# Quantum-Chemistry-Group-BNU/PyNQS

Measured on AMD Instinct MI355X. Metric: local energies/sec (whole node), higher is better.
Workload: dtype f64

## Files before the change

include/pynqs_amd.h:

```cpp
#ifndef PYNQS_AMD_H
#define PYNQS_AMD_H

#include <stdint.h>

#ifdef __cplusplus
extern "C" {
#endif

#define PYNQS_ABI_VERSION 1

#define PYNQS_OK 0
#define PYNQS_EINVAL (-1)
#define PYNQS_ELAUNCH (-2)
#define PYNQS_ELENGTH (-3)
#define PYNQS_EOVERFLOW (-4)

#define PYNQS_F32 0
#define PYNQS_F64 1

#define PYNQS_MAX_SORB_LEN 3
#define PYNQS_MAX_SORB 192
#define PYNQS_MAX_NELE 120
#define PYNQS_MAX_NVIR 120

// ... 186 lines not shown
} pynqs_reduce_io;
int pynqs_reduce_onepass_geometry(int64_t nbatch, int sorb, int nele, int noA, int noB, int eps_sample, int64_t *out4);
int64_t pynqs_reduce_onepass_tile_scratch_bytes(int64_t nbatch, int sorb, int nele, int noA, int noB, int eps_sample);
int pynqs_reduce_onepass_list_capacity(int64_t nbatch, int sorb, int nele, int noA, int noB, int dtype, int eps_sample,
                                       int with_row_cache, int without_table, int64_t *cap_doubles);
int pynqs_reduce_onepass_wants_row_f32(int64_t nbatch, int sorb, int nele, int noA, int noB, int dtype, int eps_sample, int64_t cap_doubles,
                                       int with_tile_scratch ,
                                       int without_table );
int64_t pynqs_reduce_onepass_row_f32_elements(int64_t nbatch, int sorb, int nele, int noA, int noB);
int pynqs_reduce_onepass(const uint64_t *bra, int64_t nbatch, int sorb, int nele, int noA, int noB, const void *plan,
                         int dtype, double eps, int eps_sample, uint64_t seed, const pynqs_reduce_io *io, void *stream);
int pynqs_reduce_contract(int64_t nbatch, int sorb, int nele, int noA, int noB, int dtype, int eps_sample,
                          const pynqs_reduce_io *io, const double *psi_unique, const double *psi_table, int psi_is_complex,
                          int divide, double *eloc, double *psi_x, void *stream);
#define PYNQS_CONTRACT_BATCHED 0
#define PYNQS_CONTRACT_SERIAL 1
int pynqs_reduce_contract_form(int64_t nbatch, int sorb, int nele, int noA, int noB, int dtype, int eps_sample,
                               const pynqs_reduce_io *io, const double *psi_unique, const double *psi_table, int psi_is_complex,
                               int divide, double *eloc, double *psi_x, int form, void *stream);

#define PYNQS_RBM_COMPLEX 4
int pynqs_rbm_forward(const uint64_t *onv, int64_t n, int sorb, const double *weights, const double *hidden_bias,
                      const double *visible_bias, int nhidden, int flavour, double *psi, void *stream);

int64_t pynqs_rbm_children_table_bytes(int64_t nwalkers, int sorb, int nhidden, int flavour);
int pynqs_rbm_children_prepare(const uint64_t *walkers, int64_t nwalkers, int sorb, const double *weights, const double *hidden_bias,
                               const double *visible_bias, int nhidden, int flavour, void *table, void *stream);
int pynqs_rbm_forward_children(const uint64_t *onv, int64_t n, const int32_t *count_dev, const int32_t *parent,
                               const uint64_t *walkers, int64_t nwalkers, const void *table, int sorb, const double *weights,
                               const double *hidden_bias, const double *visible_bias, int nhidden, int flavour, double *psi,
                               void *stream);
int pynqs_rbm_forward_children_supported(int sorb, int nhidden, int flavour);
int pynqs_rbm_forward_children_geometry(int64_t n, int sorb, int nhidden, int flavour, int64_t *out4);
int pynqs_rbm_children_prepare_stamped(const uint64_t *walkers, int64_t nwalkers, int sorb, const double *weights,
                                       const double *hidden_bias, const double *visible_bias, int nhidden, int flavour, uint64_t stamp,
                                       void *table, void *stream);
int pynqs_rbm_forward_children_stamped(const uint64_t *onv, int64_t n, const int32_t *count_dev, const int32_t *parent,
                                       const uint64_t *walkers, int64_t nwalkers, const void *table, int sorb, const double *weights,
                                       const double *hidden_bias, const double *visible_bias, int nhidden, int flavour, uint64_t stamp,
                                       double *psi, void *stream);

int64_t pynqs_rbm_grad_workspace(int64_t n, int sorb, int nhidden, int flavour);
int pynqs_rbm_grad(const uint64_t *onv, int64_t n, int sorb, const double *weights, const double *hidden_bias,
                   const double *visible_bias, int nhidden, int flavour, const double *prob, const double *eloc,
                   int eloc_is_complex, const double *e_total, const double *pow, double *grad_weights,
                   double *grad_hidden_bias, double *grad_visible_bias, double *loss, void *workspace, void *stream);
int pynqs_rbm_grad_loss(const uint64_t *onv, int64_t n, int sorb, const double *weights, const double *hidden_bias,
                        const double *visible_bias, int nhidden, int flavour, const double *prob, const double *eloc,
                        int eloc_is_complex, const double *e_total, const double *pow, double *grad_weights,
                        double *grad_hidden_bias, double *grad_visible_bias, double *loss, double *loss_copy, void *workspace,
                        void *stream);
#define PYNQS_GRAD_ONEPASS 0
#define PYNQS_GRAD_TWOPASS 1
int pynqs_rbm_grad_loss_form(const uint64_t *onv, int64_t n, int sorb, const double *weights, const double *hidden_bias,
                             const double *visible_bias, int nhidden, int flavour, const double *prob, const double *eloc,
                             int eloc_is_complex, const double *e_total, const double *pow, double *grad_weights,
                             double *grad_hidden_bias, double *grad_visible_bias, double *loss, double *loss_copy, void *workspace,
                             int schedule, int block, void *stream);

#define PYNQS_SR_RHO 0
#define PYNQS_SR_RHS2 1
#define PYNQS_SR_DONE 2
#define PYNQS_SR_ITER 3
#define PYNQS_SR_TRUE2 4
#define PYNQS_SR_PAP 5
#define PYNQS_SR_CONVERGED 6
#define PYNQS_SR_BREAKDOWN 7
#define PYNQS_SR_NSCALARS 8
#define PYNQS_SR_CG_INIT 0
#define PYNQS_SR_CG_STEP 1
#define PYNQS_SR_CG_RESIDUAL 2
int64_t pynqs_rbm_sr_workspace(int64_t n, int sorb, int nhidden, int flavour);
int pynqs_rbm_sr_prepare(const uint64_t *onv, int64_t n, int sorb, const double *weights, const double *hidden_bias, int nhidden,
// ... 41 lines not shown
```

pynqs_amd/C_extension.py:

```python
from __future__ import annotations

import itertools
import os
import warnings
import weakref
from typing import Tuple

import numpy as np
import torch
from torch import Tensor

from . import _native as N

MAX_SORB_LEN = 3
MAX_SORB = 64 * MAX_SORB_LEN
MAX_NELE = 120
USE_PLAN = True

__all__ = [
    "tensor_to_onv", "onv_to_tensor", "get_comb_tensor", "get_hij_torch", "get_comb_hij_fused",
    "wavefunction_lut", "hash_build", "hash_lookup", "HashTable", "RBMTable", "eloc_rbm", "JastrowTable", "eloc_jrbm", "green_jrbm", "jrbm_forward", "eloc_jrbm_supported", "merge_rank_sample", "spin_flip_rand", "check_sorb", "compress_h1e_h2e", "decompress_h1e_h2e", "get_Num_SinglesDoubles",
    "MAX_SORB", "MAX_SORB_LEN", "MAX_NELE",
]

# ... 644 lines not shown
    n = onv.size(0)
    psi = torch.empty(n, dtype=_rbm_dtype(rbm_type), device=onv.device)
    N.check(N.lib().pynqs_rbm_forward(onv.data_ptr(), n, sorb, W.data_ptr(), hb.data_ptr(), vb.data_ptr() if vb is not None else None, H, flav,
                                      psi.data_ptr(), _stream(onv.device)), "pynqs_rbm_forward")
    return psi


def _rbm_params(weights, hidden_bias, visible_bias, sorb, rbm_type, on_gpu=True):
    flav = RBM_TYPE_FLAVOUR.get(rbm_type)
    if flav is None:
        raise RuntimeError(f"rbm_type {rbm_type!r} has no fused forward")
    cplx_par = rbm_type == "complex"
    W = weights.detach().double().contiguous()
    hb = hidden_bias.detach().double().contiguous()
    vb = visible_bias.detach().double().contiguous() if visible_bias is not None else None
    H = W.size(0)
    if W.shape[:2] != (H, sorb) or W.dim() != (3 if cplx_par else 2) or hb.numel() != H * (2 if cplx_par else 1) or \
            (vb is not None and vb.numel() != sorb * (2 if cplx_par else 1)):
        raise RuntimeError("RBM parameter shapes do not match sorb / num_hidden")
    if on_gpu and not (W.is_cuda and hb.is_cuda and (vb is None or vb.is_cuda)):
        raise RuntimeError("RBM parameters must be on the GPU")
    return flav, W, hb, vb, H


def rbm_forward_children_supported(sorb: int, num_hidden: int, rbm_type: str = "real") -> bool:
    flav = RBM_TYPE_FLAVOUR.get(rbm_type)
    return flav is not None and bool(N.lib().pynqs_rbm_forward_children_supported(sorb, num_hidden, flav))


_CHILDREN_STAMP = itertools.count(1)


def rbm_forward_children(onv: Tensor, parent: Tensor, walkers: Tensor, weights: Tensor, hidden_bias: Tensor, visible_bias: "Tensor | None",
                         sorb: int, rbm_type: str = "real", count: "Tensor | None" = None, out: "Tensor | None" = None) -> Tensor:
    _check_onv(onv, "onv", sorb, (2,))
    _check_onv(walkers, "walkers", sorb, (2,))
    flav, W, hb, vb, H = _rbm_params(weights, hidden_bias, visible_bias, sorb, rbm_type)
    dev = onv.device
    if not (onv.is_cuda and walkers.device == dev and parent.device == dev and parent.dtype == torch.int32 and parent.numel() >= onv.size(0)):
        raise RuntimeError("rbm_forward_children: onv, walkers and parent (int32) on one GPU")
    n, nw = onv.size(0), walkers.size(0)
    nbytes = N.lib().pynqs_rbm_children_table_bytes(nw, sorb, H, flav)
    table = torch.empty(max(nbytes // 8, 1), dtype=torch.float64, device=dev)
    st = _stream(dev)
    wk = walkers.contiguous()
    stamp = next(_CHILDREN_STAMP)
    N.check(N.lib().pynqs_rbm_children_prepare_stamped(wk.data_ptr(), nw, sorb, W.data_ptr(), hb.data_ptr(), vb.data_ptr() if vb is not None else None,
                                                       H, flav, stamp, table.data_ptr(), st), "pynqs_rbm_children_prepare_stamped")
    psi = out if out is not None else torch.empty(n, dtype=_rbm_dtype(rbm_type), device=dev)
    N.check(N.lib().pynqs_rbm_forward_children_stamped(onv.contiguous().data_ptr(), n, count.data_ptr() if count is not None else None,
                                                       parent.data_ptr(), wk.data_ptr(), nw, table.data_ptr(), sorb, W.data_ptr(), hb.data_ptr(),
                                                       vb.data_ptr() if vb is not None else None, H, flav, stamp, psi.data_ptr(), st),
            "pynqs_rbm_forward_children_stamped")
    return psi


class CRBMTable(_RBMTableBase):

    def __init__(self, weights: Tensor, hidden_bias: Tensor, visible_bias: "Tensor | None" = None) -> None:
        def as_pairs(t: Tensor) -> Tensor:
            t = t.detach()
            if t.is_complex():
                t = torch.view_as_real(t.to(torch.complex128))
            if t.dtype != torch.float64 or t.size(-1) != 2:
                raise RuntimeError("complex RBM parameters must be complex128 or float64 (re, im) pairs")
            return t.contiguous()

        w, hb = as_pairs(weights), as_pairs(hidden_bias).reshape(-1, 2)
        vb = as_pairs(visible_bias).reshape(-1, 2) if visible_bias is not None else None
        if w.dim() != 3 or hb.size(0) != w.size(0) or (vb is not None and vb.size(0) != w.size(1)):
            raise RuntimeError("weights must be [num_hidden, sorb], hidden_bias [num_hidden], visible_bias [sorb]")
        given = [weights, hidden_bias] + ([visible_bias] if visible_bias is not None else [])
        self._build("crbm", given, [w, hb] + ([vb] if vb is not None else []), int(w.size(0)), int(w.size(1)))


def eloc_crbm(bra: Tensor, h1e: Tensor, h2e: Tensor, table: CRBMTable, sorb: int, nele: int, noA: int, noB: int,
              want_psi: bool = True, log_scale: float = 0.0) -> Tuple[Tensor, "Tensor | None"]:
    _check_onv(bra, "bra", sorb, (2,))
    return _eloc_fused(bra, h1e, h2e, table, sorb, want_psi, torch.complex128, lambda x, n, plan, eloc, psi, st: N.check(
        N.lib().pynqs_eloc_crbm(x.data_ptr(), n, sorb, nele, noA, noB, plan.data_ptr(), table.data_ptr(), table.nhidden, float(log_scale),
                                eloc.data_ptr(), psi, st), "pynqs_eloc_crbm"))


_CHARTS = None


# ... 97 lines not shown
```

pynqs_amd/_native.py:

```python
from __future__ import annotations

import ctypes as C
import os

_HERE = os.path.dirname(os.path.abspath(__file__))
LIB_PATH = os.environ.get("PYNQS_AMD_LIB") or os.path.join(_HERE, "csrc", "libpynqs_amd.so")

PYNQS_F32, PYNQS_F64 = 0, 1
RBM_REAL, RBM_TANH, RBM_PHASE, RBM_COMPLEX = 0, 1, 2, 4
OK, EINVAL, ELAUNCH, ELENGTH, EOVERFLOW = 0, -1, -2, -3, -4

_i64, _int, _vp, _dbl = C.c_int64, C.c_int, C.c_void_p, C.c_double

SIGNATURES = {
    "pynqs_abi_version": (_int, []),
    "pynqs_last_error": (C.c_char_p, []),
    "pynqs_num_sd": (_i64, [_int, _int, _int]),
    "pynqs_check_sorb": (_int, [_int, _int]),
    "pynqs_comb_hij_fused": (_int, [_vp, _i64, _int, _int, _int, _int, _vp, _vp, _int, _vp, _vp, _vp]),
    "pynqs_comb": (_int, [_vp, _i64, _int, _int, _int, _vp, _vp, _vp]),
    "pynqs_hij": (_int, [_vp, _i64, _vp, _i64, _int, _vp, _vp, _int, _int, _int, _vp, _vp]),
    "pynqs_onv_to_pm1": (_int, [_vp, _i64, _int, _int, _vp, _vp]),
    "pynqs_pm01_to_onv": (_int, [_vp, _i64, _int, _vp, _vp]),
    "pynqs_wavefunction_lut": (_int, [_vp, _i64, _vp, _i64, _int, _vp, _vp, _vp]),
    "pynqs_spin_flip_rand": (_int, [_vp, _i64, _int, _int, _int, C.c_uint64, C.c_uint64, _vp, _vp]),
    "pynqs_plan_bytes": (_i64, [_int, _int]),
    "pynqs_plan_build": (_int, [_vp, _vp, _int, _int, _vp, _vp]),
    "pynqs_comb_hij_fused_plan": (_int, [_vp, _i64, _int, _int, _int, _int, _vp, _int, _vp, _vp, _vp]),
    "pynqs_eloc_sample_space": (_int, [_vp, _i64, _int, _int, _int, _int, _vp, _vp, _i64, _vp, _int, _vp, _vp, _vp]),
    "pynqs_hash_bytes": (_i64, [_i64, _int]),
    "pynqs_hash_build": (_int, [_vp, _i64, _int, _vp, _vp]),
    "pynqs_hash_lookup": (_int, [_vp, _i64, _vp, _i64, _int, _vp, _vp, _vp]),
    "pynqs_unique_workspace": (_i64, [_i64]),
    "pynqs_unique_first": (_int, [_vp, _i64, _int, _vp, _vp, _vp]),
    "pynqs_eloc_sample_space_hash": (_int, [_vp, _i64, _int, _int, _int, _int, _vp, _vp, _i64, _vp, _int, _vp, _vp, _vp]),
    "pynqs_eloc_sample_space_flip": (_int, [_vp, _i64, _int, _int, _int, _int, _vp, _vp, _i64, _vp, _int, _vp, _vp, _vp]),
    "pynqs_eloc_sample_space_hash_flip": (_int, [_vp, _i64, _int, _int, _int, _int, _vp, _vp, _i64, _vp, _int, _vp, _vp, _vp]),
    "pynqs_eloc_sample_space_keys": (_int, [_vp, _i64, _int, _int, _int, _int, _vp, _vp, _i64, _vp, _int, _int, _vp, _vp, _vp]),
    "pynqs_keys_index_bytes": (_i64, [_i64, _int]),
    "pynqs_keys_index_workspace": (_i64, [_i64, _int]),
    "pynqs_keys_index_build": (_int, [_vp, _i64, _int, _vp, _vp, _vp]),
    "pynqs_keys_index_density": (_int, [_vp, _i64, _int, _vp, _vp]),
# ... 27 lines not shown
    "pynqs_reduce_tiles": (_i64, [_i64, _int, _int, _int, _int]),
    "pynqs_reduce_count": (_int, [_vp, _i64, _int, _int, _int, _int, _vp, _int, _dbl, _vp, _vp]),
    "pynqs_reduce_count_sums": (_int, [_vp, _i64, _int, _int, _int, _int, _vp, _int, _dbl, _vp, _vp, _vp]),
    "pynqs_reduce_sample": (_int, [_vp, _i64, _int, _int, _int, _int, _vp, _int, _dbl, _vp, _vp, _vp, C.c_uint64, _vp, _vp, _vp, _vp]),
    "pynqs_reduce_emit": (_int, [_vp, _i64, _int, _int, _int, _int, _vp, _int, _dbl, _vp, _vp, _vp, _vp, _vp]),
}



class ReduceIO(C.Structure):
    _fields_ = [("cap_doubles", _i64), ("cap_unique", _i64), ("dedup_slots", _i64),
                ("rec_col", _vp), ("rec_w", _vp), ("rec_onv", _vp), ("rec_link", _vp), ("seg_count", _vp),
                ("srec_col", _vp), ("srec_w", _vp), ("srec_onv", _vp), ("srec_link", _vp), ("row_sum", _vp),
                ("dedup_table", _vp), ("uniq_onv", _vp), ("uniq_pm1", _vp), ("pm1_dtype", C.c_int32), ("lut_is_hash", C.c_int32),
                ("lut_table", _vp), ("lut_nkeys", _i64), ("counters", _vp), ("seed_dev", _vp), ("row_cache", _vp), ("uniq_parent", _vp),
                ("tile_scratch", _vp), ("tile_scratch_bytes", _i64), ("row_f32", _vp)]


SIGNATURES.update({
    "pynqs_reduce_onepass_geometry": (_int, [_i64, _int, _int, _int, _int, _int, C.POINTER(_i64)]),
    "pynqs_reduce_onepass_tile_scratch_bytes": (_i64, [_i64, _int, _int, _int, _int, _int]),
    "pynqs_reduce_onepass_list_capacity": (_int, [_i64, _int, _int, _int, _int, _int, _int, _int, _int, C.POINTER(_i64)]),
    "pynqs_reduce_onepass_wants_row_f32": (_int, [_i64, _int, _int, _int, _int, _int, _int, _i64, _int, _int]),
    "pynqs_reduce_onepass_row_f32_elements": (_i64, [_i64, _int, _int, _int, _int]),
    "pynqs_reduce_onepass": (_int, [_vp, _i64, _int, _int, _int, _int, _vp, _int, _dbl, _int, C.c_uint64, C.POINTER(ReduceIO), _vp]),
    "pynqs_rbm_forward": (_int, [_vp, _i64, _int, _vp, _vp, _vp, _int, _int, _vp, _vp]),
    "pynqs_rbm_children_table_bytes": (_i64, [_i64, _int, _int, _int]),
    "pynqs_rbm_children_prepare": (_int, [_vp, _i64, _int, _vp, _vp, _vp, _int, _int, _vp, _vp]),
    "pynqs_rbm_forward_children": (_int, [_vp, _i64, _vp, _vp, _vp, _i64, _vp, _int, _vp, _vp, _vp, _int, _int, _vp, _vp]),
    "pynqs_rbm_forward_children_supported": (_int, [_int, _int, _int]),
    "pynqs_rbm_forward_children_geometry": (_int, [_i64, _int, _int, _int, C.POINTER(_i64)]),
    "pynqs_rbm_children_prepare_stamped": (_int, [_vp, _i64, _int, _vp, _vp, _vp, _int, _int, C.c_uint64, _vp, _vp]),
    "pynqs_rbm_forward_children_stamped": (_int, [_vp, _i64, _vp, _vp, _vp, _i64, _vp, _int, _vp, _vp, _vp, _int, _int, C.c_uint64, _vp, _vp]),
    "pynqs_rbm_grad_workspace": (_i64, [_i64, _int, _int, _int]),
    "pynqs_rbm_grad": (_int, [_vp, _i64, _int, _vp, _vp, _vp, _int, _int, _vp, _vp, _int, _vp, _vp, _vp, _vp, _vp, _vp, _vp, _vp]),
    "pynqs_rbm_grad_loss": (_int, [_vp, _i64, _int, _vp, _vp, _vp, _int, _int, _vp, _vp, _int, _vp, _vp, _vp, _vp, _vp, _vp, _vp, _vp, _vp]),
    "pynqs_rbm_grad_loss_form": (_int, [_vp, _i64, _int, _vp, _vp, _vp, _int, _int, _vp, _vp, _int, _vp, _vp, _vp, _vp, _vp, _vp, _vp, _vp, _int, _int, _vp]),
    "pynqs_reduce_contract": (_int, [_i64, _int, _int, _int, _int, _int, _int, C.POINTER(ReduceIO), _vp, _vp, _int, _int, _vp, _vp, _vp]),
    "pynqs_reduce_contract_form": (_int, [_i64, _int, _int, _int, _int, _int, _int, C.POINTER(ReduceIO), _vp, _vp, _int, _int, _vp, _vp, _int, _vp]),
    "pynqs_mcmc_rbm_supported": (_int, [_int, _int, _int]),
    "pynqs_mcmc_rbm": (_int, [_vp, _i64, _int, _int, _int, _vp, _int, _int, C.c_uint64, C.c_uint64, C.c_uint64, _int, _int, _vp, _vp, _vp, _vp]),
    "pynqs_rbm_sr_workspace": (_i64, [_i64, _int, _int, _int]),
    "pynqs_rbm_sr_prepare": (_int, [_vp, _i64, _int, _vp, _vp, _int, _int, _vp, _vp, _vp, _vp]),
    "pynqs_rbm_sr_matvec": (_int, [_vp, _i64, _int, _int, _int, _vp, _vp, _vp, _vp, _vp, _vp]),
    "pynqs_rbm_sr_cg_step": (_int, [_int, _i64, _vp, _vp, _vp, _vp, _vp, _vp, _dbl, _dbl, _dbl, _vp]),
    "pynqs_jrbm_sr_workspace": (_i64, [_i64, _int, _int]),
    "pynqs_jrbm_sr_prepare": (_int, [_vp, _i64, _int, _vp, _vp, _int, _vp, _vp, _vp, _vp]),
    "pynqs_jrbm_sr_matvec": (_int, [_vp, _i64, _int, _int, _vp, _vp, _vp, _vp, _vp, _vp]),
    "pynqs_mcmc_accept": (_int, [_vp, _vp, _vp, _vp, _i64, _int, _int, C.c_uint64, C.c_uint64, C.c_uint64, _vp, _vp, _vp]),
    "pynqs_rdm_scatter": (_int, [_vp, _i64, _int, _int, _int, _int, _vp, _vp, _int, _vp, _vp, _vp]),
    "pynqs_rdm_rbm_supported": (_int, [_int, _int, _int, _int, _int]),
    "pynqs_rdm_rbm_workspace": (_i64, [_i64, _int, _int]),
    "pynqs_rdm_rbm": (_int, [_vp, _i64, _int, _int, _int, _int, _vp, _vp, _int, _vp, _vp, _vp, _vp]),
    "pynqs_rdm_jrbm_supported": (_int, [_int, _int, _int, _int, _int]),
    "pynqs_rdm_jrbm_workspace": (_i64, [_i64, _int, _int]),
    "pynqs_rdm_jrbm": (_int, [_vp, _i64, _int, _int, _int, _int, _vp, _vp, _vp, _int, _vp, _vp, _vp, _vp]),
    "pynqs_jastrow_table_bytes": (_i64, [_int]),
    "pynqs_jastrow_table_build": (_int, [_vp, _int, _vp, _vp]),
    "pynqs_eloc_jrbm_supported": (_int, [_int, _int, _int, _int, _int]),
    "pynqs_eloc_jrbm_form": (_int, [_i64, _int, _int, _int, _int, _int]),
    "pynqs_eloc_jrbm": (_int, [_vp, _i64, _int, _int, _int, _int, _vp, _vp, _vp, _int, _vp, _vp, _vp]),
    "pynqs_eloc_jrbm_flip_supported": (_int, [_int, _int, _int, _int, _int]),
    "pynqs_eloc_jrbm_flip_form": (_int, [_i64, _int, _int, _int, _int, _int]),
    "pynqs_eloc_jrbm_signed": (_int, [_vp, _i64, _int, _int, _int, _int, _vp, _vp, _vp, _int, _vp, _vp, _vp]),
    "pynqs_eloc_jrbm_flip": (_int, [_vp, _i64, _int, _int, _int, _int, _vp, _vp, _vp, _vp, _vp, _int, _dbl, _dbl, _vp, _vp, _vp, _vp, _vp]),
    "pynqs_green_jrbm": (_int, [_vp, _i64, _int, _int, _int, _int, _vp, _vp, _vp, _int, _dbl, _vp, _vp, _vp, _vp, _vp]),
# ... 47 lines not shown
```

pynqs_amd/csrc/kernels_rbm_forward.hip:

```cpp
#include "detcore.h"
#include "launch.h"
#include "rbm_math.h"

namespace pynqs {

constexpr int kHChunk = 8;

struct Prod {
  double re = 1.0, im = 0.0;
  double lin = 0.0, ang = 0.0;
  int e2 = 0;
  __device__ __forceinline__ void renorm() {
    int k;
    (void)frexp(fmax(fabs(re), fabs(im)), &k);
    re = ldexp(re, -k); im = ldexp(im, -k);
    e2 += k;
  }
  __device__ __forceinline__ bool finite() const { return fabs(re) < __builtin_inf() && fabs(im) < __builtin_inf(); }
  template <bool CPLX>
  __device__ __forceinline__ void times_2cosh(double x, double y) {
    const double ax = fabs(x);
    const double rho = exp(-2.0 * ax);
    lin += ax;
    if constexpr (CPLX) {
      const double sy = x < 0.0 ? -y : y;
      double sn, cs;
      sincos_mod(-2.0 * sy, sn, cs);
      const double u = fma(rho, cs, 1.0), v = rho * sn;
      const double nr = re * u - im * v;
      im = fma(re, v, im * u);
      re = nr;
      ang += sy;
    } else {
      re *= 1.0 + rho;
    }
  }
};

template <int FLAVOUR>
__device__ __forceinline__ void write_psi(double *__restrict__ psi, int64_t i, const Prod &P, double axr, double axi) {
  const double kLn2 = 0.693147180559945309417;
  if constexpr (FLAVOUR == PYNQS_RBM_REAL) {
    psi[i] = P.re * exp(axr + P.lin + kLn2 * (double)P.e2);
  } else if constexpr (FLAVOUR == PYNQS_RBM_TANH) {
    psi[i] = tanh(axr) * P.re * exp(P.lin + kLn2 * (double)P.e2);
  } else if constexpr (FLAVOUR == PYNQS_RBM_PHASE) {
    double sn, cs;
    sincos(axr + P.lin + log(P.re) + kLn2 * (double)P.e2, &sn, &cs);
    psi[2 * i] = cs; psi[2 * i + 1] = sn;
  } else {
    const double m = exp(axr + P.lin + kLn2 * (double)P.e2);
    double sn, cs;
    sincos(axi + P.ang, &sn, &cs);
    psi[2 * i] = m * (P.re * cs - P.im * sn);
    psi[2 * i + 1] = m * (P.re * sn + P.im * cs);
  }
}

template <int LEN, int FLAVOUR>
__device__ __forceinline__ void rbm_forward_row(const uint64_t (&ket)[LEN], int sorb, int H, const double *__restrict__ W,
                                                const double *__restrict__ hb, const double *__restrict__ vb, Prod &P, double &axr, double &axi) {
  constexpr bool CPLX = FLAVOUR == PYNQS_RBM_COMPLEX;
  for (int h0 = 0; h0 < H; h0 += kHChunk) {
    double tr[kHChunk], ti[kHChunk];
#pragma unroll
    for (int j = 0; j < kHChunk; ++j) {
      const int h = min(h0 + j, H - 1);
      tr[j] = CPLX ? hb[2 * h] : hb[h];
      ti[j] = CPLX ? hb[2 * h + 1] : 0.0;
    }
    for (int o = 0; o < sorb; ++o) {
      const double x = pm1_of<LEN>(ket, o);
#pragma unroll
      for (int j = 0; j < kHChunk; ++j) {
        const int h = min(h0 + j, H - 1);
        if constexpr (CPLX) {
          tr[j] = fma(x, W[((size_t)h * sorb + o) * 2], tr[j]);
          ti[j] = fma(x, W[((size_t)h * sorb + o) * 2 + 1], ti[j]);
        } else {
          tr[j] = fma(x, W[(size_t)h * sorb + o], tr[j]);
        }
      }
    }
#pragma unroll
    for (int j = 0; j < kHChunk; ++j)
      if (h0 + j < H) P.template times_2cosh<CPLX>(tr[j], ti[j]);
    P.renorm();
  }
// ... 196 lines not shown
  const int64_t i = (int64_t)blockIdx.x * kBlock + threadIdx.x;
  if ((int64_t)blockIdx.x * kBlock >= n) return;
  const int64_t row = i < n ? i : n - 1;
  uint64_t ket[LEN];
#pragma unroll
  for (int w = 0; w < LEN; ++w) ket[w] = onv[row * LEN + w];
  double *__restrict__ out = table + (size_t)row * (size_t)(H + 2) * C;
  if ((int)blockIdx.y < nchunks) {
    children_parent_chunk<LEN, CPLX>(ket, i < n, (int)blockIdx.y * kParentChunk, sorb, H, W, hb,
                                     factors + (size_t)(2 * sorb + 1) * children_hp(H) * C, stamp, out);
    return;
  }
  for (int o = threadIdx.x; o < sorb; o += kBlock) {
    double re, im;
    sum_w_column<CPLX>(W, sorb, H, o, re, im);
    fs[o][0][0] = re * 2.0;
    fs[o][1][0] = vb ? 2.0 * vb[(size_t)o * C] : 0.0;
    if constexpr (CPLX) {
      fs[o][0][1] = im * 2.0;
      fs[o][1][1] = vb ? 2.0 * vb[(size_t)o * C + 1] : 0.0;
    }
  }
  __syncthreads();
  children_parent_sums<LEN, CPLX>(ket, i < n, sorb, H, hb, &fs[0][0][0], (size_t)2 * C, out);
}

__device__ __forceinline__ bool children_flag_raised(double word, double stamp) { return stamp != 0.0 ? word == stamp : word != 0.0; }

#ifndef PYNQS_CHILD_BLOCK
#define PYNQS_CHILD_BLOCK 1024
#endif
constexpr int kChildBlock = PYNQS_CHILD_BLOCK;
constexpr int kChildWaveRows = 16;
constexpr int64_t kChildMaxBlocks = 1024;
constexpr int64_t kChildMaxWaveBlocks = 256 * 32;

template <int LEN, int FLAVOUR>
__global__ __launch_bounds__(kChildBlock) void rbm_forward_children_kernel(const uint64_t *__restrict__ onv, int64_t n, const int32_t *__restrict__ count_dev,
                                                                      const int32_t *__restrict__ parent, const uint64_t *__restrict__ walkers,
                                                                      int64_t nwalkers, const double *__restrict__ table,
                                                                      const double *__restrict__ factors, int sorb, int H,
                                                                      const double *__restrict__ W, const double *__restrict__ hb,
                                                                      const double *__restrict__ vb, double *__restrict__ psi, double stamp) {
  constexpr bool CPLX = FLAVOUR == PYNQS_RBM_COMPLEX;
  constexpr int C = CPLX ? 2 : 1;
  extern __shared__ __attribute__((aligned(16))) double wl[];
  const int HP = children_hp(H);
  int64_t cnt = n;
  if (count_dev) cnt = min((int64_t)max(*count_dev, 0), n);
  if (children_flag_raised(factors[(size_t)(2 * sorb + 1) * HP * C], stamp)) {
    const int64_t rounds = (cnt + (int64_t)gridDim.x * kChildBlock - 1) / ((int64_t)gridDim.x * kChildBlock);
    for (int64_t r = 0; r < rounds; ++r) {
      const int64_t i = ((int64_t)r * gridDim.x + blockIdx.x) * kChildBlock + threadIdx.x;
      const int64_t row = i < cnt ? i : cnt - 1;
      uint64_t ket[LEN];
#pragma unroll
      for (int w = 0; w < LEN; ++w) ket[w] = onv[row * LEN + w];
      Prod P;
      double axr, axi;
      rbm_forward_row<LEN, FLAVOUR>(ket, sorb, H, W, hb, vb, P, axr, axi);
      if (i < cnt) write_psi<FLAVOUR>(psi, i, P, axr, axi);
    }
    return;
  }
  for (int idx = threadIdx.x; idx < (2 * sorb + 1) * HP * C; idx += kChildBlock) wl[idx] = factors[idx];
  __syncthreads();
  for (int64_t i = (int64_t)blockIdx.x * kChildBlock + threadIdx.x; i < cnt; i += (int64_t)gridDim.x * kChildBlock) {
    int64_t p = parent[i];
    bool stranger = p < 0 || p >= nwalkers;
    p = stranger ? 0 : p;
    int at[4];
#pragma unroll
    for (int q = 0; q < 4; ++q) at[q] = 2 * sorb * HP;
    int k = 0, nflip = 0;
#pragma unroll
    for (int w = 0; w < LEN; ++w) {
      const uint64_t xc = onv[i * LEN + w];
      uint64_t d = xc ^ walkers[p * LEN + w];
      nflip += __popcll(d);
#pragma unroll
      for (int t = 0; t < 4; ++t) {
        if (d && k < 4) {
          const int b = __builtin_ctzll(d);
          d &= d - 1;
          const int r = (2 * (64 * w + b) + (((xc >> b) & 1ull) ? 0 : 1)) * HP;
#pragma unroll
          for (int q = 0; q < 4; ++q)
            if (q == k) at[q] = r;
          ++k;
        }
      }
    }
    const double *__restrict__ tp = table + (size_t)p * (size_t)(H + 2) * C;
    Prod P;
    for (int h0 = 0; h0 < H; h0 += kHChunk) {
#pragma unroll
      for (int j = 0; j < kHChunk; ++j) {
        const int h = h0 + j;
        if (h < H) {
          double qr = tp[(size_t)h * C], qi = CPLX ? tp[(size_t)h * C + 1] : 0.0;
#pragma unroll
          for (int q = 0; q < 4; ++q) {
            const double fr = wl[(size_t)(at[q] + h) * C];
            if constexpr (CPLX) {
              const double fi = wl[(size_t)(at[q] + h) * C + 1];
              const double nr = qr * fr - qi * fi;
              qi = fma(qr, fi, qi * fr);
              qr = nr;
            } else {
              qr *= fr;
            }
          }
          if constexpr (CPLX) {
            const double u = 1.0 + qr;
            const double nr = P.re * u - P.im * qi;
            P.im = fma(P.re, qi, P.im * u);
            P.re = nr;
          } else {
            P.re *= 1.0 + qr;
          }
        }
      }
      P.renorm();
    }
    double axr = tp[(size_t)(H + 1) * C], axi = CPLX ? tp[(size_t)(H + 1) * C + 1] : 0.0;
    P.lin = tp[(size_t)H * C];
    P.ang = CPLX ? tp[(size_t)H * C + 1] : 0.0;
#pragma unroll
    for (int q = 0; q < 4; ++q) {
      P.lin += wl[(size_t)(at[q] + H) * C];
      axr += wl[(size_t)(at[q] + H + 1) * C];
      if constexpr (CPLX) {
        P.ang += wl[(size_t)(at[q] + H) * C + 1];
        axi += wl[(size_t)(at[q] + H + 1) * C + 1];
      }
    }
    stranger = stranger || nflip > 4 || !P.finite();
    if (__ballot(stranger)) {
      uint64_t ket[LEN];
#pragma unroll
      for (int w = 0; w < LEN; ++w) ket[w] = onv[i * LEN + w];
      Prod P2;
      double a2r, a2i;
      rbm_forward_row<LEN, FLAVOUR>(ket, sorb, H, W, hb, vb, P2, a2r, a2i);
      if (stranger) { P = P2; axr = a2r; axi = a2i; }
    }
    write_psi<FLAVOUR>(psi, i, P, axr, axi);
  }
}

template <int LEN, int FLAVOUR>
__global__ __launch_bounds__(kBlock) void rbm_forward_children_wave_kernel(const uint64_t *__restrict__ onv, int64_t n, const int32_t *__restrict__ count_dev,
                                                                           const int32_t *__restrict__ parent, const uint64_t *__restrict__ walkers,
                                                                           int64_t nwalkers, const double *__restrict__ table,
                                                                           const double *__restrict__ factors, int sorb, int H,
                                                                           const double *__restrict__ W, const double *__restrict__ hb,
                                                                           const double *__restrict__ vb, double *__restrict__ psi, double stamp) {
  constexpr bool CPLX = FLAVOUR == PYNQS_RBM_COMPLEX;
  constexpr int C = CPLX ? 2 : 1;
  const int HP = children_hp(H);
  int64_t cnt = n;
  if (count_dev) cnt = min((int64_t)max(*count_dev, 0), n);
  if (children_flag_raised(factors[(size_t)(2 * sorb + 1) * HP * C], stamp)) {
    const int64_t rounds = (cnt + (int64_t)gridDim.x * kBlock - 1) / ((int64_t)gridDim.x * kBlock);
    for (int64_t r = 0; r < rounds; ++r) {
      const int64_t i = ((int64_t)r * gridDim.x + blockIdx.x) * kBlock + threadIdx.x;
      const int64_t row = i < cnt ? i : cnt - 1;
      uint64_t ket[LEN];
#pragma unroll
      for (int w = 0; w < LEN; ++w) ket[w] = onv[row * LEN + w];
      Prod P;
      double axr, axi;
      rbm_forward_row<LEN, FLAVOUR>(ket, sorb, H, W, hb, vb, P, axr, axi);
      if (i < cnt) write_psi<FLAVOUR>(psi, i, P, axr, axi);
    }
    return;
  }
  const int lane = threadIdx.x & 63;
  const int wave = __builtin_amdgcn_readfirstlane((int)(threadIdx.x >> 6));
  const int64_t nwaves = (int64_t)gridDim.x * (kBlock / 64);
// ... 233 lines not shown
  int64_t blocks, table_rows, scratch_rows;
};
static ChildrenGeometry children_geometry(int64_t n, int sorb, int nhidden, int flavour) {
  ChildrenGeometry g;
  g.in_lds = children_table_in_lds(sorb, nhidden, flavour);
  if (g.in_lds) {
    g.blocks = (n + kChildBlock - 1) / kChildBlock;
    if (g.blocks > kChildMaxBlocks) g.blocks = kChildMaxBlocks;
    g.table_rows = g.scratch_rows = g.blocks * kChildBlock;
  } else {
    constexpr int64_t rows = (kBlock / 64) * kChildWaveRows;
    g.blocks = (n + rows - 1) / rows;
    if (g.blocks > kChildMaxWaveBlocks) g.blocks = kChildMaxWaveBlocks;
    g.table_rows = g.blocks * rows;
    g.scratch_rows = g.blocks * kBlock;
  }
  return g;
}

extern "C" int pynqs_rbm_forward_children_geometry(int64_t n, int sorb, int nhidden, int flavour, int64_t *out4) {
  if (!out4) return set_error(PYNQS_EINVAL, "null pointer");
  if (n < 0 || n > 0x7fffffffll * kBlock || !pynqs_rbm_forward_children_supported(sorb, nhidden, flavour))
    return set_error(PYNQS_EINVAL, "rbm_forward_children_geometry: bad n/sorb/nhidden/flavour");
  const ChildrenGeometry g = children_geometry(n, sorb, nhidden, flavour);
  out4[0] = g.in_lds ? 0 : 1;
  out4[1] = g.blocks;
  out4[2] = g.table_rows;
  out4[3] = g.scratch_rows;
  return PYNQS_OK;
}

static int forward_children_launch(const uint64_t *onv, int64_t n, const int32_t *count_dev, const int32_t *parent, const uint64_t *walkers,
                                   int64_t nwalkers, const void *table, int sorb, const double *weights, const double *hidden_bias,
                                   const double *visible_bias, int nhidden, int flavour, double stamp, double *psi, void *stream) {
  pynqs::DeviceScope device_scope_(onv);
  if (n < 0 || n > 0x7fffffffll * kBlock || nwalkers < 0 || sorb < 1 || sorb > kMaxSorb || nhidden < 1) return set_error(PYNQS_EINVAL, "bad n/sorb/nhidden");
  if (!pynqs_rbm_forward_children_supported(sorb, nhidden, flavour))
    return set_error(PYNQS_EINVAL, "rbm_forward_children: bad flavour");
  if (n == 0) return PYNQS_OK;
  if (!onv || !parent || !walkers || !table || !psi || !weights || !hidden_bias || nwalkers == 0) return set_error(PYNQS_EINVAL, "null pointer");
  const int len = (sorb - 1) / 64 + 1;
  const ChildrenGeometry geo = children_geometry(n, sorb, nhidden, flavour);
  const uint32_t grid = (uint32_t)geo.blocks;
  const size_t lds = children_lds_bytes(sorb, nhidden, flavour);
  const double *parents = (const double *)table;
  const double *factors = parents + (size_t)nwalkers * (size_t)(nhidden + 2) * (flavour == PYNQS_RBM_COMPLEX ? 2 : 1);
  hipStream_t st = (hipStream_t)stream;
  const bool in_lds = geo.in_lds;
#define PYNQS_RC(F)                                                                                                                          \
  do {                                                                                                                                       \
    if (in_lds)                                                                                                                              \
      hipLaunchKernelGGL((rbm_forward_children_kernel<LEN, F>), dim3(grid), dim3(kChildBlock), lds, st, onv, n, count_dev, parent, walkers,  \
                         nwalkers, parents, factors, sorb, nhidden, weights, hidden_bias, visible_bias, psi, stamp);                         \
    else                                                                                                                                     \
      hipLaunchKernelGGL((rbm_forward_children_wave_kernel<LEN, F>), dim3(grid), dim3(kBlock), 0, st, onv, n, count_dev,                     \
                         parent, walkers, nwalkers, parents, factors, sorb, nhidden, weights, hidden_bias, visible_bias, psi, stamp);        \
  } while (0)
  DISPATCH_LEN(len, {
    switch (flavour) {
      case PYNQS_RBM_REAL: PYNQS_RC(PYNQS_RBM_REAL); break;
      case PYNQS_RBM_TANH: PYNQS_RC(PYNQS_RBM_TANH); break;
      case PYNQS_RBM_PHASE: PYNQS_RC(PYNQS_RBM_PHASE); break;
      default: PYNQS_RC(PYNQS_RBM_COMPLEX); break;
    }
  });
#undef PYNQS_RC
  return check_launch("rbm_forward_children");
}

extern "C" int pynqs_rbm_forward_children(const uint64_t *onv, int64_t n, const int32_t *count_dev, const int32_t *parent,
                                          const uint64_t *walkers, int64_t nwalkers, const void *table, int sorb, const double *weights,
                                          const double *hidden_bias, const double *visible_bias, int nhidden, int flavour, double *psi,
                                          void *stream) {
  return forward_children_launch(onv, n, count_dev, parent, walkers, nwalkers, table, sorb, weights, hidden_bias, visible_bias, nhidden, flavour,
                                 0.0, psi, stream);
}

extern "C" int pynqs_rbm_forward_children_stamped(const uint64_t *onv, int64_t n, const int32_t *count_dev, const int32_t *parent,
                                                  const uint64_t *walkers, int64_t nwalkers, const void *table, int sorb, const double *weights,
                                                  const double *hidden_bias, const double *visible_bias, int nhidden, int flavour,
                                                  uint64_t stamp, double *psi, void *stream) {
  if (!children_stamp_ok(stamp)) return set_error(PYNQS_EINVAL, "rbm_forward_children_stamped: stamp must be in [1, 2^53)");
  return forward_children_launch(onv, n, count_dev, parent, walkers, nwalkers, table, sorb, weights, hidden_bias, visible_bias, nhidden, flavour,
                                 (double)stamp, psi, stream);
}
```

Baseline: 10.16 million.

## Restructure RBM children kernel with chunked double-buffered hidden loop and vector LDS fill

Rewrites the RBM children forward kernel so each row walks the hidden units in chunks held in registers, double-buffering the parent-table loads (real case) and grouping the factor loads from LDS. The LDS factor fill now uses staged double2 loads, the grid cap drops from 1024 to 256 blocks, and fallback rows are recomputed from scratch in a separate pass. A form selector (chunked by default, per-unit via an env var) is exposed through new C entry points. Explicit fma and rounded ops keep the arithmetic ordering deterministic, but the extra register pressure and the smaller grid may hurt occupancy.

```diff
diff --git a/include/pynqs_amd.h b/include/pynqs_amd.h
--- a/include/pynqs_amd.h
+++ b/include/pynqs_amd.h
@@ -242,6 +242,12 @@
                                void *stream);
 int pynqs_rbm_forward_children_supported(int sorb, int nhidden, int flavour);
 int pynqs_rbm_forward_children_geometry(int64_t n, int sorb, int nhidden, int flavour, int64_t *out4);
+#define PYNQS_CHILDREN_CHUNKED 0
+#define PYNQS_CHILDREN_PER_UNIT 1
+int pynqs_rbm_forward_children_form(const uint64_t *onv, int64_t n, const int32_t *count_dev, const int32_t *parent,
+                                    const uint64_t *walkers, int64_t nwalkers, const void *table, int sorb, const double *weights,
+                                    const double *hidden_bias, const double *visible_bias, int nhidden, int flavour, int form, double *psi,
+                                    void *stream);
 int pynqs_rbm_children_prepare_stamped(const uint64_t *walkers, int64_t nwalkers, int sorb, const double *weights,
                                        const double *hidden_bias, const double *visible_bias, int nhidden, int flavour, uint64_t stamp,
                                        void *table, void *stream);
@@ -249,6 +255,10 @@
                                        const uint64_t *walkers, int64_t nwalkers, const void *table, int sorb, const double *weights,
                                        const double *hidden_bias, const double *visible_bias, int nhidden, int flavour, uint64_t stamp,
                                        double *psi, void *stream);
+int pynqs_rbm_forward_children_stamped_form(const uint64_t *onv, int64_t n, const int32_t *count_dev, const int32_t *parent,
+                                            const uint64_t *walkers, int64_t nwalkers, const void *table, int sorb, const double *weights,
+                                            const double *hidden_bias, const double *visible_bias, int nhidden, int flavour, uint64_t stamp,
+                                            int form, double *psi, void *stream);
 
 int64_t pynqs_rbm_grad_workspace(int64_t n, int sorb, int nhidden, int flavour);
 int pynqs_rbm_grad(const uint64_t *onv, int64_t n, int sorb, const double *weights, const double *hidden_bias,
diff --git a/pynqs_amd/C_extension.py b/pynqs_amd/C_extension.py
--- a/pynqs_amd/C_extension.py
+++ b/pynqs_amd/C_extension.py
@@ -700,7 +700,10 @@
 
 
 def rbm_forward_children(onv: Tensor, parent: Tensor, walkers: Tensor, weights: Tensor, hidden_bias: Tensor, visible_bias: "Tensor | None",
-                         sorb: int, rbm_type: str = "real", count: "Tensor | None" = None, out: "Tensor | None" = None) -> Tensor:
+                         sorb: int, rbm_type: str = "real", count: "Tensor | None" = None, out: "Tensor | None" = None,
+                         form: "int | None" = None) -> Tensor:
+    if form is None:
+        form = N.CHILDREN_PER_UNIT if os.environ.get("PYNQS_RBM_CHILDREN_FORM") == "1" else N.CHILDREN_CHUNKED
     _check_onv(onv, "onv", sorb, (2,))
     _check_onv(walkers, "walkers", sorb, (2,))
     flav, W, hb, vb, H = _rbm_params(weights, hidden_bias, visible_bias, sorb, rbm_type)
@@ -716,10 +719,11 @@
     N.check(N.lib().pynqs_rbm_children_prepare_stamped(wk.data_ptr(), nw, sorb, W.data_ptr(), hb.data_ptr(), vb.data_ptr() if vb is not None else None,
                                                        H, flav, stamp, table.data_ptr(), st), "pynqs_rbm_children_prepare_stamped")
     psi = out if out is not None else torch.empty(n, dtype=_rbm_dtype(rbm_type), device=dev)
-    N.check(N.lib().pynqs_rbm_forward_children_stamped(onv.contiguous().data_ptr(), n, count.data_ptr() if count is not None else None,
-                                                       parent.data_ptr(), wk.data_ptr(), nw, table.data_ptr(), sorb, W.data_ptr(), hb.data_ptr(),
-                                                       vb.data_ptr() if vb is not None else None, H, flav, stamp, psi.data_ptr(), st),
-            "pynqs_rbm_forward_children_stamped")
+    N.check(N.lib().pynqs_rbm_forward_children_stamped_form(onv.contiguous().data_ptr(), n, count.data_ptr() if count is not None else None,
+                                                            parent.data_ptr(), wk.data_ptr(), nw, table.data_ptr(), sorb, W.data_ptr(),
+                                                            hb.data_ptr(), vb.data_ptr() if vb is not None else None, H, flav, stamp, int(form),
+                                                            psi.data_ptr(), st),
+            "pynqs_rbm_forward_children_stamped_form")
     return psi
 
 
diff --git a/pynqs_amd/_native.py b/pynqs_amd/_native.py
--- a/pynqs_amd/_native.py
+++ b/pynqs_amd/_native.py
@@ -8,6 +8,7 @@
 
 PYNQS_F32, PYNQS_F64 = 0, 1
 RBM_REAL, RBM_TANH, RBM_PHASE, RBM_COMPLEX = 0, 1, 2, 4
+CHILDREN_CHUNKED, CHILDREN_PER_UNIT = 0, 1
 OK, EINVAL, ELAUNCH, ELENGTH, EOVERFLOW = 0, -1, -2, -3, -4
 
 _i64, _int, _vp, _dbl = C.c_int64, C.c_int, C.c_void_p, C.c_double
@@ -101,6 +102,8 @@
     "pynqs_rbm_forward_children_geometry": (_int, [_i64, _int, _int, _int, C.POINTER(_i64)]),
     "pynqs_rbm_children_prepare_stamped": (_int, [_vp, _i64, _int, _vp, _vp, _vp, _int, _int, C.c_uint64, _vp, _vp]),
     "pynqs_rbm_forward_children_stamped": (_int, [_vp, _i64, _vp, _vp, _vp, _i64, _vp, _int, _vp, _vp, _vp, _int, _int, C.c_uint64, _vp, _vp]),
+    "pynqs_rbm_forward_children_form": (_int, [_vp, _i64, _vp, _vp, _vp, _i64, _vp, _int, _vp, _vp, _vp, _int, _int, _int, _vp, _vp]),
+    "pynqs_rbm_forward_children_stamped_form": (_int, [_vp, _i64, _vp, _vp, _vp, _i64, _vp, _int, _vp, _vp, _vp, _int, _int, C.c_uint64, _int, _vp, _vp]),
     "pynqs_rbm_grad_workspace": (_i64, [_i64, _int, _int, _int]),
     "pynqs_rbm_grad": (_int, [_vp, _i64, _int, _vp, _vp, _vp, _int, _int, _vp, _vp, _int, _vp, _vp, _vp, _vp, _vp, _vp, _vp, _vp]),
     "pynqs_rbm_grad_loss": (_int, [_vp, _i64, _int, _vp, _vp, _vp, _int, _int, _vp, _vp, _int, _vp, _vp, _vp, _vp, _vp, _vp, _vp, _vp, _vp]),
diff --git a/pynqs_amd/csrc/kernels_rbm_forward.hip b/pynqs_amd/csrc/kernels_rbm_forward.hip
--- a/pynqs_amd/csrc/kernels_rbm_forward.hip
+++ b/pynqs_amd/csrc/kernels_rbm_forward.hip
@@ -39,6 +39,7 @@
 
 template <int FLAVOUR>
 __device__ __forceinline__ void write_psi(double *__restrict__ psi, int64_t i, const Prod &P, double axr, double axi) {
+#pragma clang fp contract(off)
   const double kLn2 = 0.693147180559945309417;
   if constexpr (FLAVOUR == PYNQS_RBM_REAL) {
     psi[i] = P.re * exp(axr + P.lin + kLn2 * (double)P.e2);
@@ -52,8 +53,8 @@
     const double m = exp(axr + P.lin + kLn2 * (double)P.e2);
     double sn, cs;
     sincos(axi + P.ang, &sn, &cs);
-    psi[2 * i] = m * (P.re * cs - P.im * sn);
-    psi[2 * i + 1] = m * (P.re * sn + P.im * cs);
+    psi[2 * i] = m * fma(P.re, cs, -(P.im * sn));
+    psi[2 * i + 1] = m * fma(P.re, sn, P.im * cs);
   }
 }
 
@@ -316,10 +317,175 @@
 #endif
 constexpr int kChildBlock = PYNQS_CHILD_BLOCK;
 constexpr int kChildWaveRows = 16;
-constexpr int64_t kChildMaxBlocks = 1024;
+#ifndef PYNQS_CHILD_MAX_BLOCKS
+#define PYNQS_CHILD_MAX_BLOCKS 256
+#endif
+constexpr int64_t kChildMaxBlocks = PYNQS_CHILD_MAX_BLOCKS;
 constexpr int64_t kChildMaxWaveBlocks = 256 * 32;
 
+template <bool CPLX>
+__device__ __forceinline__ void children_times_factor(double &qr, double &qi, double fr, double fi) {
+  if constexpr (CPLX) {
+    const double t = __dmul_rn(qi, fi);
+    const double nr = fma(qr, fr, -t);
+    qi = fma(qr, fi, __dmul_rn(qi, fr));
+    qr = nr;
+  } else {
+    qr = __dmul_rn(qr, fr);
+  }
+}
+template <bool CPLX>
+__device__ __forceinline__ void children_times_one_plus(Prod &P, double qr, double qi, double fr, double fi) {
+  if constexpr (CPLX) {
+    children_times_factor<true>(qr, qi, fr, fi);
+    const double u = __dadd_rn(qr, 1.0);
+    const double t = __dmul_rn(P.im, qi);
+    const double nr = fma(P.re, u, -t);
+    P.im = fma(P.re, qi, __dmul_rn(P.im, u));
+    P.re = nr;
+  } else {
+    P.re = __dmul_rn(P.re, fma(qr, fr, 1.0));
+  }
+}
+
+constexpr int kChildGroupCplx = 4;
+template <bool CPLX>
+struct ChildQ {
+  double v[kHChunk][CPLX ? 2 : 1];
+};
+template <bool CPLX>
+__device__ __forceinline__ void children_load_q(const double *__restrict__ tp, int h0, ChildQ<CPLX> &q) {
+  constexpr int C = CPLX ? 2 : 1;
+#pragma unroll
+  for (int j = 0; j < kHChunk; ++j)
+#pragma unroll
+    for (int c = 0; c < C; ++c) q.v[j][c] = tp[(size_t)(h0 + j) * C + c];
+}
+
+template <bool CPLX>
+__device__ __forceinline__ void children_chunk(Prod &P, ChildQ<CPLX> &q, const double *__restrict__ wl, const int (&at)[4], int h0) {
+  constexpr int C = CPLX ? 2 : 1;
+  constexpr int G = CPLX ? kChildGroupCplx : kHChunk;
+#pragma unroll
+  for (int s = 0; s < 4; ++s) {
+#pragma unroll
+    for (int g = 0; g < kHChunk; g += G) {
+      double f[G][C];
+#pragma unroll
+      for (int j = 0; j < G; ++j)
+#pragma unroll
+        for (int c = 0; c < C; ++c) f[j][c] = wl[(size_t)(at[s] + h0 + g + j) * C + c];
+#pragma unroll
+      for (int j = 0; j < G; ++j) {
+        double zero = 0.0;
+        double &qi = CPLX ? q.v[g + j][C - 1] : zero;
+        const double fi = CPLX ? f[j][C - 1] : 0.0;
+        if (s < 3) children_times_factor<CPLX>(q.v[g + j][0], qi, f[j][0], fi);
+        else children_times_one_plus<CPLX>(P, q.v[g + j][0], qi, f[j][0], fi);
+      }
+    }
+  }
+  P.renorm();
+}
+
 template <int LEN, int FLAVOUR>
+__device__ __forceinline__ void children_row_from_scratch(const uint64_t *__restrict__ onv, int64_t row, int sorb, int H,
+                                                       const double *__restrict__ W, const double *__restrict__ hb,
+                                                       const double *__restrict__ vb, Prod &P, double &axr, double &axi) {
+  uint64_t ket[LEN];
+#pragma unroll
+  for (int w = 0; w < LEN; ++w) ket[w] = onv[row * LEN + w];
+  P = Prod();
+  rbm_forward_row<LEN, FLAVOUR>(ket, sorb, H, W, hb, vb, P, axr, axi);
+}
+
+template <int LEN, bool CPLX, int FORM>
+__device__ __forceinline__ bool children_row_from_table(const uint64_t *__restrict__ onv, int64_t i, const int32_t *__restrict__ parent,
+                                                        const uint64_t *__restrict__ walkers, int64_t nwalkers,
+                                                        const double *__restrict__ table, const double *__restrict__ wl, int sorb, int H,
+                                                        Prod &P, double &axr, double &axi) {
+  constexpr int C = CPLX ? 2 : 1;
+  const int HP = children_hp(H);
+  int64_t p = parent[i];
+  bool stranger = p < 0 || p >= nwalkers;
+  p = stranger ? 0 : p;
+  const double *__restrict__ tp = table + (size_t)p * (size_t)(H + 2) * C;
+  constexpr bool kChunked = FORM == PYNQS_CHILDREN_CHUNKED;
+  const int hfull = kChunked ? H - H % kHChunk : 0;
+  ChildQ<CPLX> qa;
+  if (hfull > 0) children_load_q<CPLX>(tp, 0, qa);
+  int at[4];
+#pragma unroll
+  for (int q = 0; q < 4; ++q) at[q] = 2 * sorb * HP;
+  int k = 0, nflip = 0;
+#pragma unroll
+  for (int w = 0; w < LEN; ++w) {
+    const uint64_t xc = onv[i * LEN + w];
+    uint64_t d = xc ^ walkers[p * LEN + w];
+    nflip += __popcll(d);
+#pragma unroll
+    for (int t = 0; t < 4; ++t) {
+      if (d && k < 4) {
+        const int b = __builtin_ctzll(d);
+        d &= d - 1;
+        const int r = (2 * (64 * w + b) + (((xc >> b) & 1ull) ? 0 : 1)) * HP;
+#pragma unroll
+        for (int q = 0; q < 4; ++q)
+          if (q == k) at[q] = r;
+        ++k;
+      }
+    }
+  }
+  P = Prod();
+  if constexpr (!CPLX) {
+    ChildQ<CPLX> qb;
+    for (int h0 = 0; h0 < hfull; h0 += 2 * kHChunk) {
+      if (h0 + kHChunk < hfull) children_load_q<CPLX>(tp, h0 + kHChunk, qb);
+      children_chunk<CPLX>(P, qa, wl, at, h0);
+      if (h0 + kHChunk >= hfull) break;
+      if (h0 + 2 * kHChunk < hfull) children_load_q<CPLX>(tp, h0 + 2 * kHChunk, qa);
+      children_chunk<CPLX>(P, qb, wl, at, h0 + kHChunk);
+    }
+  } else {
+    for (int h0 = 0; h0 < hfull; h0 += kHChunk) {
+      if (h0 > 0) children_load_q<CPLX>(tp, h0, qa);
+      children_chunk<CPLX>(P, qa, wl, at, h0);
+    }
+  }
+  for (int h0 = hfull; h0 < H; h0 += kHChunk) {
+#pragma unroll
+    for (int j = 0; j < kHChunk; ++j) {
+      const int h = h0 + j;
+      if (h < H) {
+        double qr = tp[(size_t)h * C], qi = CPLX ? tp[(size_t)h * C + 1] : 0.0;
+#pragma unroll
+        for (int q = 0; q < 3; ++q)
+          children_times_factor<CPLX>(qr, qi, wl[(size_t)(at[q] + h) * C], CPLX ? wl[(size_t)(at[q] + h) * C + 1] : 0.0);
+        children_times_one_plus<CPLX>(P, qr, qi, wl[(size_t)(at[3] + h) * C], CPLX ? wl[(size_t)(at[3] + h) * C + 1] : 0.0);
+      }
+    }
+    P.renorm();
+  }
+  axr = tp[(size_t)(H + 1) * C];
+  axi = CPLX ? tp[(size_t)(H + 1) * C + 1] : 0.0;
+  P.lin = tp[(size_t)H * C];
+  P.ang = CPLX ? tp[(size_t)H * C + 1] : 0.0;
+#pragma unroll
+  for (int q = 0; q < 4; ++q) {
+    P.lin += wl[(size_t)(at[q] + H) * C];
+    axr += wl[(size_t)(at[q] + H + 1) * C];
+    if constexpr (CPLX) {
+      P.ang += wl[(size_t)(at[q] + H) * C + 1];
+      axi += wl[(size_t)(at[q] + H + 1) * C + 1];
+    }
+  }
+  return stranger || nflip > 4 || !P.finite();
+}
+
+constexpr int kChildStage = 4;
+constexpr long long kChildAgainBits = 0x7ff8c41d5eedc41dll;
+
+template <int LEN, int FLAVOUR, int FORM>
 __global__ __launch_bounds__(kChildBlock) void rbm_forward_children_kernel(const uint64_t *__restrict__ onv, int64_t n, const int32_t *__restrict__ count_dev,
                                                                       const int32_t *__restrict__ parent, const uint64_t *__restrict__ walkers,
                                                                       int64_t nwalkers, const double *__restrict__ table,
@@ -328,108 +494,51 @@
                                                                       const double *__restrict__ vb, double *__restrict__ psi, double stamp) {
   constexpr bool CPLX = FLAVOUR == PYNQS_RBM_COMPLEX;
   constexpr int C = CPLX ? 2 : 1;
+  constexpr int CO = (CPLX || FLAVOUR == PYNQS_RBM_PHASE) ? 2 : 1;
   extern __shared__ __attribute__((aligned(16))) double wl[];
   const int HP = children_hp(H);
   int64_t cnt = n;
   if (count_dev) cnt = min((int64_t)max(*count_dev, 0), n);
-  if (children_flag_raised(factors[(size_t)(2 * sorb + 1) * HP * C], stamp)) {
-    const int64_t rounds = (cnt + (int64_t)gridDim.x * kChildBlock - 1) / ((int64_t)gridDim.x * kChildBlock);
-    for (int64_t r = 0; r < rounds; ++r) {
-      const int64_t i = ((int64_t)r * gridDim.x + blockIdx.x) * kChildBlock + threadIdx.x;
-      const int64_t row = i < cnt ? i : cnt - 1;
-      uint64_t ket[LEN];
-#pragma unroll
-      for (int w = 0; w < LEN; ++w) ket[w] = onv[row * LEN + w];
+  const int64_t first = (int64_t)blockIdx.x * kChildBlock + threadIdx.x, stride = (int64_t)gridDim.x * kChildBlock;
+  const bool raised = children_flag_raised(factors[(size_t)(2 * sorb + 1) * HP * C], stamp);
+  bool again = raised;
+  if (!raised) {
+    const int total = (2 * sorb + 1) * HP * C;
+    const int head = (int)(((uintptr_t)factors >> 3) & 1);
+    const int nvec = (total - head) >> 1;
+    const double2 *__restrict__ src = reinterpret_cast<const double2 *>(factors + head);
+    for (int base = threadIdx.x; base < nvec; base += kChildBlock * kChildStage) {
+      double2 v[kChildStage];
+#pragma unroll
+      for (int b = 0; b < kChildStage; ++b) v[b] = src[min(base + b * kChildBlock, nvec - 1)];
+#pragma unroll
+      for (int b = 0; b < kChildStage; ++b) {
+        const int idx = base + b * kChildBlock;
+        if (idx < nvec) { wl[head + 2 * idx] = v[b].x; wl[head + 2 * idx + 1] = v[b].y; }
+      }
+    }
+    if (threadIdx.x == 0 && head) wl[0] = factors[0];
+    if (threadIdx.x == 64 % kChildBlock && head + 2 * nvec < total) wl[total - 1] = factors[total - 1];
+    __syncthreads();
+    for (int64_t i = first; i < cnt; i += stride) {
       Prod P;
       double axr, axi;
-      rbm_forward_row<LEN, FLAVOUR>(ket, sorb, H, W, hb, vb, P, axr, axi);
-      if (i < cnt) write_psi<FLAVOUR>(psi, i, P, axr, axi);
-    }
-    return;
-  }
-  for (int idx = threadIdx.x; idx < (2 * sorb + 1) * HP * C; idx += kChildBlock) wl[idx] = factors[idx];
-  __syncthreads();
-  for (int64_t i = (int64_t)blockIdx.x * kChildBlock + threadIdx.x; i < cnt; i += (int64_t)gridDim.x * kChildBlock) {
-    int64_t p = parent[i];
-    bool stranger = p < 0 || p >= nwalkers;
-    p = stranger ? 0 : p;
-    int at[4];
-#pragma unroll
-    for (int q = 0; q < 4; ++q) at[q] = 2 * sorb * HP;
-    int k = 0, nflip = 0;
-#pragma unroll
-    for (int w = 0; w < LEN; ++w) {
-      const uint64_t xc = onv[i * LEN + w];
-      uint64_t d = xc ^ walkers[p * LEN + w];
-      nflip += __popcll(d);
-#pragma unroll
-      for (int t = 0; t < 4; ++t) {
-        if (d && k < 4) {
-          const int b = __builtin_ctzll(d);
-          d &= d - 1;
-          const int r = (2 * (64 * w + b) + (((xc >> b) & 1ull) ? 0 : 1)) * HP;
-#pragma unroll
-          for (int q = 0; q < 4; ++q)
-            if (q == k) at[q] = r;
-          ++k;
-        }
-      }
-    }
-    const double *__restrict__ tp = table + (size_t)p * (size_t)(H + 2) * C;
+      if (children_row_from_table<LEN, CPLX, FORM>(onv, i, parent, walkers, nwalkers, table, wl, sorb, H, P, axr, axi)) {
+        again = true;
+        psi[CO * i] = __longlong_as_double(kChildAgainBits);
+      } else {
+        write_psi<FLAVOUR>(psi, i, P, axr, axi);
+      }
+    }
+  }
+  if (!__ballot(again)) return;
+  for (int64_t i = first; i < cnt; i += stride) {
+    const bool mine = raised || (again && __double_as_longlong(psi[CO * i]) == kChildAgainBits);
+    if (!__ballot(mine)) continue;
     Prod P;
-    for (int h0 = 0; h0 < H; h0 += kHChunk) {
-#pragma unroll
-      for (int j = 0; j < kHChunk; ++j) {
-        const int h = h0 + j;
-        if (h < H) {
-          double qr = tp[(size_t)h * C], qi = CPLX ? tp[(size_t)h * C + 1] : 0.0;
-#pragma unroll
-          for (int q = 0; q < 4; ++q) {
-            const double fr = wl[(size_t)(at[q] + h) * C];
-            if constexpr (CPLX) {
-              const double fi = wl[(size_t)(at[q] + h) * C + 1];
-              const double nr = qr * fr - qi * fi;
-              qi = fma(qr, fi, qi * fr);
-              qr = nr;
-            } else {
-              qr *= fr;
-            }
-          }
-          if constexpr (CPLX) {
-            const double u = 1.0 + qr;
-            const double nr = P.re * u - P.im * qi;
-            P.im = fma(P.re, qi, P.im * u);
-            P.re = nr;
-          } else {
-            P.re *= 1.0 + qr;
-          }
-        }
-      }
-      P.renorm();
-    }
-    double axr = tp[(size_t)(H + 1) * C], axi = CPLX ? tp[(size_t)(H + 1) * C + 1] : 0.0;
-    P.lin = tp[(size_t)H * C];
-    P.ang = CPLX ? tp[(size_t)H * C + 1] : 0.0;
-#pragma unroll
-    for (int q = 0; q < 4; ++q) {
-      P.lin += wl[(size_t)(at[q] + H) * C];
-      axr += wl[(size_t)(at[q] + H + 1) * C];
-      if constexpr (CPLX) {
-        P.ang += wl[(size_t)(at[q] + H) * C + 1];
-        axi += wl[(size_t)(at[q] + H + 1) * C + 1];
-      }
-    }
-    stranger = stranger || nflip > 4 || !P.finite();
-    if (__ballot(stranger)) {
-      uint64_t ket[LEN];
-#pragma unroll
-      for (int w = 0; w < LEN; ++w) ket[w] = onv[i * LEN + w];
-      Prod P2;
-      double a2r, a2i;
-      rbm_forward_row<LEN, FLAVOUR>(ket, sorb, H, W, hb, vb, P2, a2r, a2i);
-      if (stranger) { P = P2; axr = a2r; axi = a2i; }
-    }
-    write_psi<FLAVOUR>(psi, i, P, axr, axi);
+    double axr, axi;
+    children_row_from_scratch<LEN, FLAVOUR>(onv, i, sorb, H, W, hb, vb, P, axr, axi);
+    if (mine) write_psi<FLAVOUR>(psi, i, P, axr, axi);
   }
 }
 
@@ -729,8 +838,9 @@
 
 static int forward_children_launch(const uint64_t *onv, int64_t n, const int32_t *count_dev, const int32_t *parent, const uint64_t *walkers,
                                    int64_t nwalkers, const void *table, int sorb, const double *weights, const double *hidden_bias,
-                                   const double *visible_bias, int nhidden, int flavour, double stamp, double *psi, void *stream) {
+                                   const double *visible_bias, int nhidden, int flavour, double stamp, int form, double *psi, void *stream) {
   pynqs::DeviceScope device_scope_(onv);
+  if (form != PYNQS_CHILDREN_CHUNKED && form != PYNQS_CHILDREN_PER_UNIT) return set_error(PYNQS_EINVAL, "rbm_forward_children: bad form");
   if (n < 0 || n > 0x7fffffffll * kBlock || nwalkers < 0 || sorb < 1 || sorb > kMaxSorb || nhidden < 1) return set_error(PYNQS_EINVAL, "bad n/sorb/nhidden");
   if (!pynqs_rbm_forward_children_supported(sorb, nhidden, flavour))
     return set_error(PYNQS_EINVAL, "rbm_forward_children: bad flavour");
@@ -746,9 +856,14 @@
   const bool in_lds = geo.in_lds;
 #define PYNQS_RC(F)                                                                                                                          \
   do {                                                                                                                                       \
-    if (in_lds)                                                                                                                              \
-      hipLaunchKernelGGL((rbm_forward_children_kernel<LEN, F>), dim3(grid), dim3(kChildBlock), lds, st, onv, n, count_dev, parent, walkers,  \
-                         nwalkers, parents, factors, sorb, nhidden, weights, hidden_bias, visible_bias, psi, stamp);                         \
+    if (in_lds && form == PYNQS_CHILDREN_CHUNKED)                                                                                            \
+      hipLaunchKernelGGL((rbm_forward_children_kernel<LEN, F, PYNQS_CHILDREN_CHUNKED>), dim3(grid), dim3(kChildBlock), lds, st, onv, n,      \
+                         count_dev, parent, walkers, nwalkers, parents, factors, sorb, nhidden, weights, hidden_bias, visible_bias, psi,     \
+                         stamp);                                                                                                             \
+    else if (in_lds)                                                                                                                         \
+      hipLaunchKernelGGL((rbm_forward_children_kernel<LEN, F, PYNQS_CHILDREN_PER_UNIT>), dim3(grid), dim3(kChildBlock), lds, st, onv, n,     \
+                         count_dev, parent, walkers, nwalkers, parents, factors, sorb, nhidden, weights, hidden_bias, visible_bias, psi,     \
+                         stamp);                                                                                                             \
     else                                                                                                                                     \
       hipLaunchKernelGGL((rbm_forward_children_wave_kernel<LEN, F>), dim3(grid), dim3(kBlock), 0, st, onv, n, count_dev,                     \
                          parent, walkers, nwalkers, parents, factors, sorb, nhidden, weights, hidden_bias, visible_bias, psi, stamp);        \
@@ -765,19 +880,35 @@
   return check_launch("rbm_forward_children");
 }
 
+extern "C" int pynqs_rbm_forward_children_form(const uint64_t *onv, int64_t n, const int32_t *count_dev, const int32_t *parent,
+                                               const uint64_t *walkers, int64_t nwalkers, const void *table, int sorb, const double *weights,
+                                               const double *hidden_bias, const double *visible_bias, int nhidden, int flavour, int form,
+                                               double *psi, void *stream) {
+  return forward_children_launch(onv, n, count_dev, parent, walkers, nwalkers, table, sorb, weights, hidden_bias, visible_bias, nhidden, flavour,
+                                 0.0, form, psi, stream);
+}
+
 extern "C" int pynqs_rbm_forward_children(const uint64_t *onv, int64_t n, const int32_t *count_dev, const int32_t *parent,
                                           const uint64_t *walkers, int64_t nwalkers, const void *table, int sorb, const double *weights,
                                           const double *hidden_bias, const double *visible_bias, int nhidden, int flavour, double *psi,
                                           void *stream) {
+  return pynqs_rbm_forward_children_form(onv, n, count_dev, parent, walkers, nwalkers, table, sorb, weights, hidden_bias, visible_bias, nhidden,
+                                         flavour, PYNQS_CHILDREN_CHUNKED, psi, stream);
+}
+
+extern "C" int pynqs_rbm_forward_children_stamped_form(const uint64_t *onv, int64_t n, const int32_t *count_dev, const int32_t *parent,
+                                                       const uint64_t *walkers, int64_t nwalkers, const void *table, int sorb,
+                                                       const double *weights, const double *hidden_bias, const double *visible_bias,
+                                                       int nhidden, int flavour, uint64_t stamp, int form, double *psi, void *stream) {
+  if (!children_stamp_ok(stamp)) return set_error(PYNQS_EINVAL, "rbm_forward_children_stamped: stamp must be in [1, 2^53)");
   return forward_children_launch(onv, n, count_dev, parent, walkers, nwalkers, table, sorb, weights, hidden_bias, visible_bias, nhidden, flavour,
-                                 0.0, psi, stream);
+                                 (double)stamp, form, psi, stream);
 }
 
 extern "C" int pynqs_rbm_forward_children_stamped(const uint64_t *onv, int64_t n, const int32_t *count_dev, const int32_t *parent,
                                                   const uint64_t *walkers, int64_t nwalkers, const void *table, int sorb, const double *weights,
                                                   const double *hidden_bias, const double *visible_bias, int nhidden, int flavour,
                                                   uint64_t stamp, double *psi, void *stream) {
-  if (!children_stamp_ok(stamp)) return set_error(PYNQS_EINVAL, "rbm_forward_children_stamped: stamp must be in [1, 2^53)");
-  return forward_children_launch(onv, n, count_dev, parent, walkers, nwalkers, table, sorb, weights, hidden_bias, visible_bias, nhidden, flavour,
-                                 (double)stamp, psi, stream);
-}
+  return pynqs_rbm_forward_children_stamped_form(onv, n, count_dev, parent, walkers, nwalkers, table, sorb, weights, hidden_bias, visible_bias,
+                                                 nhidden, flavour, stamp, PYNQS_CHILDREN_CHUNKED, psi, stream);
+}
```

New measurement: 10.42 million, median of 6. 1.03x the previous value.
